# femto-dev/femto

Hardware: AMD Instinct MI355X
Metric: patterns/sec (count+locate) on 1 GiB index (higher is better)
Workload: dtype int64

## Files before the change

femto_amd/__init__.py:

```python
import ctypes as C
import os

import numpy as np

from . import build as _build

__all__ = ["Index", "Extractor", "FemtoAmdError", "lib", "ALPHA_SIZE", "CHARACTER_OFFSET", "Info"]

ALPHA_SIZE = 261
CHARACTER_OFFSET = 5
ERR_NAMES = {0: "NOERR", 1: "MEM", 2: "IO", 3: "PARAM", 4: "FORMAT", 5: "BZ_DATA", 6: "INVALID",
             8: "MISSING", 10: "FULL", 11: "OVERWORKED", 12: "UNKNOWN"}
ERR_PARAM, ERR_INVALID, ERR_FULL, ERR_OVERWORKED = 3, 6, 10, 11
BUDGET_ALL = -2


class FemtoAmdError(RuntimeError):
    def __init__(self, code, msg):
        super().__init__(f"femto_amd error {code} ({ERR_NAMES.get(code, '?')}): {msg}")
        self.code = code


class Info(C.Structure):
    _fields_ = [("total_length", C.c_int64), ("number_of_blocks", C.c_int64), ("number_of_documents", C.c_int64),
# ... 48 lines not shown
            v = lib().femto_amd_regexp_nfa(h).contents
            n, t = v.num_nodes, v.num_transitions

            def arr(p, count, ct):
                return np.ctypeslib.as_array(C.cast(p, C.POINTER(ct)), shape=(count,)).copy() if count else np.zeros(0, dtype=ct)

            return cls(arr(v.trans_start, n + 1, C.c_int32), arr(v.trans_char, t, C.c_int32), arr(v.trans_dest, t, C.c_int32),
                       arr(v.is_start, n, C.c_uint8), arr(v.is_final, n, C.c_uint8),
                       (v.cost_bound, v.subst_cost, v.delete_cost, v.insert_cost))
        finally:
            lib().femto_amd_regexp_free(h)

    @classmethod
    def from_query(cls, query, icase=False, streamline=True):
        q = np.frombuffer(bytes(query) + b"\0", dtype=np.uint8)
        h = C.c_void_p()
        _check(lib().femto_amd_query_compile(_ptr(q), len(query), (1 if icase else 0) | (0 if streamline else 2), C.byref(h)))
        try:
            v = lib().femto_amd_regexp_nfa(h).contents
            n, t = v.num_nodes, v.num_transitions

            def arr(p, count, ct):
                return np.ctypeslib.as_array(C.cast(p, C.POINTER(ct)), shape=(count,)).copy() if count else np.zeros(0, dtype=ct)

            a = cls(arr(v.trans_start, n + 1, C.c_int32), arr(v.trans_char, t, C.c_int32), arr(v.trans_dest, t, C.c_int32),
                    arr(v.is_start, n, C.c_uint8), arr(v.is_final, n, C.c_uint8),
                    (v.cost_bound, v.subst_cost, v.delete_cost, v.insert_cost))
            sp, sn = C.c_void_p(), C.c_int64(0)
            lit = None
            if lib().femto_amd_regexp_literal(h, C.byref(sp), C.byref(sn)):
                lit = arr(sp, sn.value, C.c_uint16)
            return a, lit, lib().femto_amd_regexp_echo(h)
        finally:
            lib().femto_amd_regexp_free(h)

    def struct(self):
        return NfaStruct(self.num_nodes, len(self.trans_char), self.trans_start.ctypes.data, self.trans_char.ctypes.data,
                         self.trans_dest.ctypes.data, self.is_start.ctypes.data, self.is_final.ctypes.data, *self.settings)


class NfaBatch:

    def __init__(self, nfas):
        self.nfas = list(nfas)
        self.n = len(self.nfas)
        self.arr = (NfaStruct * max(1, self.n))(*[a.struct() for a in self.nfas])


_lib = None


def lib():
    global _lib
    if _lib is None:
        if not os.path.exists(_build.LIB):
            raise ImportError(f"{_build.LIB} is missing: run `python -c 'import __graft_entry__ as g; g.build()'` "
                              "(there is no CPU fallback)")
        import sys
        if "torch" not in sys.modules:
            try:
                import torch
            except ImportError:
                pass
        L = C.CDLL(_build.LIB)
        vp, i64, i32 = C.c_void_p, C.c_int64, C.c_int
        L.femto_amd_open.argtypes = [C.c_char_p, i32, C.POINTER(vp)]
        L.femto_amd_close.argtypes = [vp]
        L.femto_amd_close.restype = None
        L.femto_amd_last_error.restype = C.c_char_p
        L.femto_amd_info.argtypes = [vp, C.POINTER(Info)]
        L.femto_amd_count_flat.argtypes = [vp, i64, vp, vp, vp, vp, vp]
        L.femto_amd_count_bytes.argtypes = [vp, i64, vp, vp, vp, vp, vp]
        L.femto_amd_locate_flat.argtypes = [vp, i64, vp, vp, vp, i32, vp, vp, vp, i64, C.POINTER(i64)]
        L.femto_amd_locate_flat_alloc.argtypes = [vp, i64, vp, vp, vp, i32, vp, vp, C.POINTER(vp), C.POINTER(i64)]
        L.femto_amd_parallel_locate_range.argtypes = [vp, i64, i64, vp]
        L.femto_amd_parallel_count.argtypes = [vp, i32, vp, vp, vp, vp]
        L.femto_amd_parallel_locate.argtypes = [vp, i32, vp, vp, i32, vp, vp]
        L.femto_amd_resolve_location.argtypes = [vp, i64, C.POINTER(i64), C.POINTER(i64)]
        L.femto_amd_document_info.argtypes = [vp, i64, C.POINTER(C.c_char_p), C.POINTER(i64)]
        L.femto_amd_count_device.argtypes = [vp, i64, vp, vp, vp, vp, vp, vp]
        L.femto_amd_locate_plan_device.argtypes = [vp, i64, vp, vp, vp, i32, vp, vp, vp, vp, vp]
        L.femto_amd_locate_walk_device.argtypes = [vp, i64, vp, vp, i64, vp, vp]
        L.femto_amd_locate_device.argtypes = [vp, i64, vp, vp, vp, i32, vp, vp, vp, vp, vp, i64, vp, vp]
        L.femto_amd_pack_counts_device.argtypes = [vp, i64, vp, vp, vp, vp, i64, vp, vp]
        L.femto_amd_trace_lines.argtypes = [vp, i64, vp, vp, vp, i32, vp, vp, C.POINTER(i64)]
        L.femto_amd_open_multi.argtypes = [C.c_char_p, i32, vp, C.POINTER(vp)]
        L.femto_amd_open_multi_striped.argtypes = [C.c_char_p, i32, vp, C.POINTER(vp)]
        L.femto_amd_striped_serve.argtypes = [vp, C.c_char_p, i32]
        L.femto_amd_open_striped_client.argtypes = [C.c_char_p, C.c_char_p, i32, i32, C.POINTER(vp)]
        L.femto_amd_multi_child.argtypes = [vp, i32, C.POINTER(vp)]
        L.femto_amd_device_count.argtypes = [vp]
        L.femto_amd_comm_unique_id.argtypes = [vp]
        L.femto_amd_comm_init.argtypes = [vp, vp, i32, i32]
        L.femto_amd_comm_gather.argtypes = [vp, vp, vp, i64, i32, vp]
        L.femto_amd_comm_info.argtypes = [vp, C.POINTER(i32), C.POINTER(i32)]
        L.femto_amd_regexp_search.argtypes = [vp, vp, i64, i64, vp, vp, vp, C.POINTER(i64)]
        L.femto_amd_regexp_search_approx.argtypes = [vp, vp, i64, i32, i32, i32, i32, i64, vp, vp, vp, vp, C.POINTER(i64)]
        L.femto_amd_regexp_match.argtypes = [vp, i64, vp, i64]
        L.femto_amd_options_init.argtypes = [vp]
        L.femto_amd_options_init.restype = None
        L.femto_amd_open_opts.argtypes = [C.c_char_p, i32, vp, C.POINTER(vp)]
        L.femto_amd_host_pipeline_stats.argtypes = [vp, vp]
        L.femto_amd_key_format.argtypes = [vp, C.POINTER(i32), C.POINTER(i32), vp]
        L.femto_amd_pack_keys_device.argtypes = [vp, i64, vp, vp, vp, vp, vp, vp]
        L.femto_amd_locate_keys_device.argtypes = [vp, i64, vp, i32, vp, vp, vp, vp, vp, vp, i64, vp, vp]
        L.femto_amd_regexp_compile.argtypes = [vp, i64, i32, i32, i32, i32, C.POINTER(vp)]
        L.femto_amd_regexp_nfa.argtypes = [vp]
        L.femto_amd_regexp_nfa.restype = C.POINTER(NfaStruct)
        L.femto_amd_regexp_free.argtypes = [vp]
        L.femto_amd_regexp_free.restype = None
        L.femto_amd_nfa_search_batch.argtypes = [vp, i64, vp, i64, vp, vp, vp, vp, vp, vp, C.POINTER(i64)]
        L.femto_amd_nfa_stats.argtypes = [vp, vp]
        if hasattr(L, "femto_amd_lf_steps_device"):
            L.femto_amd_lf_steps_device.argtypes = [vp, i64, vp, vp, vp, vp]
        L.femto_amd_key_table_id.argtypes = [vp, C.POINTER(C.c_uint64)]
        L.femto_amd_set_option.argtypes = [vp, C.c_char_p, i32]
        L.femto_amd_block_requests.argtypes = [vp, i64, vp, vp, vp, vp, vp]
        L.femto_amd_kernel_time_ms.argtypes = [vp, C.c_char_p, C.POINTER(C.c_double), C.POINTER(i64)]
        L.femto_amd_kernel_time_reset.argtypes = [vp]
        L.femto_amd_kernel_time_reset.restype = None
        L.femto_amd_kernel_time_enable.argtypes = [vp, i32]
        L.femto_amd_kernel_time_enable.restype = None
        L.femto_amd_build_index.argtypes = [C.c_char_p, i32, vp, vp, vp, C.c_char_p, i32]
        L.femto_amd_build_index_from_sa.argtypes = [C.c_char_p, i32, vp, vp, vp, C.c_char_p, vp]
        L.femto_amd_forward_steps.argtypes = [vp, i64, vp, vp, vp, vp]
        L.femto_amd_resolve_batch.argtypes = [vp, i64, vp, vp, vp]
        L.femto_amd_resolve_device.argtypes = [vp, vp, i64, vp, vp, vp, vp, vp]
        L.femto_amd_query_compile.argtypes = [vp, i64, i32, C.POINTER(vp)]
        L.femto_amd_regexp_literal.argtypes = [vp, C.POINTER(vp), C.POINTER(i64)]
        L.femto_amd_regexp_echo.argtypes = [vp]
        L.femto_amd_regexp_echo.restype = C.c_char_p
        L.femto_amd_query_echo.argtypes = [vp, i64, i32, i32, vp, i64]
        L.femto_amd_set_rank_mode.argtypes = [vp, i32]
        L.femto_amd_get_rank_mode.argtypes = [vp]
        L.femto_amd_pack_info.argtypes = [vp, C.POINTER(i32), C.POINTER(i64), C.POINTER(C.c_double), C.POINTER(i32)]
        L.femto_amd_structures.argtypes = [vp, vp, i32]
        L.femto_amd_flatten_index.argtypes = [C.c_char_p, C.c_char_p]
        L.femto_amd_bseq_encode.argtypes = [vp, i64, i32, vp, i64, C.POINTER(i64)]
        L.femto_amd_open_split.argtypes = [C.c_char_p, i32, i32, i32, C.POINTER(vp)]
        L.femto_amd_split_export.argtypes = [vp, vp]
        L.femto_amd_split_attach.argtypes = [vp, i32, vp]
        L.femto_amd_split_attach_local.argtypes = [vp, vp]
        L.femto_amd_split_commit.argtypes = [vp]
        L.femto_amd_split_info.argtypes = [vp, C.POINTER(i32), C.POINTER(i32), C.POINTER(i64), C.POINTER(i64)]
        L.femto_amd_extractor_open.argtypes = [vp, i32, i32, C.POINTER(vp)]
        L.femto_amd_extractor_free.argtypes = [vp]
        L.femto_amd_extractor_free.restype = None
        L.femto_amd_extractor_info.argtypes = [vp, C.POINTER(i32), C.POINTER(i32), C.POINTER(i64), C.POINTER(C.c_double)]
        L.femto_amd_extractor_eof_rows.argtypes = [vp, vp, i64]
        L.femto_amd_extract_device.argtypes = [vp, i64, vp, vp, vp, vp, vp]
        L.femto_amd_context_device.argtypes = [vp, i64, vp, vp, vp, i32, i32, vp, vp, vp]
        L.femto_amd_extract.argtypes = [vp, i64, vp, vp, vp, vp]
        L.femto_amd_context.argtypes = [vp, i64, vp, vp, i32, i32, vp, vp]
        L.femto_amd_extract_document.argtypes = [vp, i64, C.POINTER(vp), C.POINTER(i64)]
        L.femto_amd_doclist_info.argtypes = [C.POINTER(i32), C.POINTER(i32)]
        L.femto_amd_doclist_device.argtypes = [vp, i64, vp, vp, i64, vp, vp, vp, vp, vp, vp, vp, vp, vp, vp]
        L.femto_amd_docset_device.argtypes = [vp, i64, vp, vp, vp, vp, vp, vp, vp, vp, vp, i64, vp, vp]
        L.femto_amd_doclist.argtypes = [vp, i64, vp, vp, vp, i32, vp, C.POINTER(vp), C.POINTER(vp), C.POINTER(i64)]
        L.femto_amd_docset.argtypes = [vp, i64, vp, vp, vp, vp, vp, vp, vp, vp, C.POINTER(vp), C.POINTER(i64)]
        L.femto_amd_docpos_info.argtypes = [C.POINTER(i32)]
        L.femto_amd_docpos_device.argtypes = [vp, i64, vp, vp, vp, vp, vp, vp, vp, vp, vp, vp, vp, vp, vp, i64, vp, vp]
        L.femto_amd_docpos_documents_device.argtypes = [vp, i64, vp, vp, vp, vp, i64, vp, vp]
        L.femto_amd_docpos.argtypes = [vp, i64, vp, vp, vp, vp, vp, vp, vp, vp, vp, vp, vp, C.POINTER(vp), C.POINTER(vp), C.POINTER(i64)]
        L.femto_amd_proximity.argtypes = [vp, i64, vp, vp, vp, vp, vp, vp, vp, vp, i32, vp, C.POINTER(vp), C.POINTER(vp), C.POINTER(i64)]
        L.femto_amd_bquery_compile.argtypes = [vp, i64, i32, C.POINTER(vp)]
        L.femto_amd_bquery_info.argtypes = [vp, C.POINTER(i32), C.POINTER(i32), C.POINTER(i32)]
# ... 303 lines not shown
    def _pairs_back(n, res_starts, pd, po, total):
        if not total.value:
            return res_starts, np.zeros(0, dtype=np.int64), np.zeros(0, dtype=np.int64)
        try:
            return (res_starts, np.ctypeslib.as_array(C.cast(pd, C.POINTER(C.c_int64)), shape=(total.value,)).copy(),
                    np.ctypeslib.as_array(C.cast(po, C.POINTER(C.c_int64)), shape=(total.value,)).copy())
        finally:
            _libc_free(pd)
            _libc_free(po)

    def docpos(self, a_lists, b_lists, ops, distances):
        n = len(ops)

        def pack(lists):
            arrs = [np.asarray(x, dtype=np.int64).reshape(-1, 2) for x in lists]
            ln = np.array([len(x) for x in arrs], dtype=np.int32)
            st = np.zeros(n, dtype=np.int64)
            if n:
                st[1:] = np.cumsum(ln[:-1], dtype=np.int64)
            flat = np.concatenate(arrs) if n and ln.sum() else np.zeros((1, 2), dtype=np.int64)
            return np.ascontiguousarray(flat[:, 0]), np.ascontiguousarray(flat[:, 1]), st, ln

        (ad, ao, sa, na), (bd, bo, sb, nb) = pack(a_lists), pack(b_lists)
        op = np.ascontiguousarray(ops, dtype=np.int32)
        di = np.ascontiguousarray(distances, dtype=np.int32)
        res_starts = np.zeros(n + 1, dtype=np.int64)
        pd, po, total = C.c_void_p(), C.c_void_p(), C.c_int64(0)
        _check(lib().femto_amd_docpos(self._h, n, _ptr(ad), _ptr(ao), _ptr(sa), _ptr(na), _ptr(bd), _ptr(bo), _ptr(sb), _ptr(nb), _ptr(op),
                                      _ptr(di), _ptr(res_starts), C.byref(pd), C.byref(po), C.byref(total)))
        return self._pairs_back(n, res_starts, pd, po, total)

    def proximity(self, left, right, ops, distances, max_occs):
        n = len(ops)
        lp, lf, ls = flatten(left)
        rp, rf, rs = flatten(right)
        op = np.ascontiguousarray(ops, dtype=np.int32)
        di = np.ascontiguousarray(distances, dtype=np.int32)
        res_starts = np.zeros(n + 1, dtype=np.int64)
        pd, po, total = C.c_void_p(), C.c_void_p(), C.c_int64(0)
        _check(lib().femto_amd_proximity(self._h, n, _ptr(lp), _ptr(lf), _ptr(ls), _ptr(rp), _ptr(rf), _ptr(rs), _ptr(op), _ptr(di),
                                         int(max_occs), _ptr(res_starts), C.byref(pd), C.byref(po), C.byref(total)))
        return self._pairs_back(n, res_starts, pd, po, total)

    def bquery_run_batch(self, queries, max_occs):
        n = len(queries)
        handles = (C.c_void_p * max(1, n))(*[q._h for q in queries])
        res_starts = np.zeros(n + 1, dtype=np.int64)
        res_type = np.zeros(max(1, n), dtype=np.int32)
        pd, po, total = C.c_void_p(), C.c_void_p(), C.c_int64(0)
        _check(lib().femto_amd_bquery_run_batch(self._h, n, C.cast(handles, C.c_void_p), int(max_occs), _ptr(res_starts), _ptr(res_type),
                                                C.byref(pd), C.byref(po), C.byref(total)))
        return (res_starts, res_type[:n]) + self._pairs_back(n, res_starts, pd, po, total)[1:]

    def docpos_device(self, npairs, d_a_doc, d_a_off, d_a_start, d_a_n, d_b_doc, d_b_off, d_b_start, d_b_n, d_op, d_distance, d_res_starts,
                      d_res_doc, d_res_off, res_capacity, d_res_total, stream=0):
        _check(lib().femto_amd_docpos_device(self._h, int(npairs), d_a_doc or None, d_a_off or None, d_a_start or None, d_a_n or None,
                                             d_b_doc or None, d_b_off or None, d_b_start or None, d_b_n or None, d_op or None,
                                             d_distance or None, d_res_starts or None, d_res_doc or None, d_res_off or None,
                                             int(res_capacity), d_res_total or None, stream or None))

    def docpos_documents_device(self, nlists, d_starts, d_pair_doc, d_doc_starts, d_docs, doc_capacity, d_total, stream=0):
        _check(lib().femto_amd_docpos_documents_device(self._h, int(nlists), d_starts or None, d_pair_doc or None, d_doc_starts or None,
                                                       d_docs or None, int(doc_capacity), d_total or None, stream or None))

    def count_device(self, npats, d_plen, d_pats, d_starts, d_first, d_last, stream=0):
        _check(lib().femto_amd_count_device(self._h, npats, d_plen, d_pats, d_starts, d_first, d_last or None,
                                            stream or None))

    def locate_plan_device(self, npats, d_plen, d_pats, d_starts, max_occs, d_first, d_last, d_noccs, d_out_starts,
                           stream=0):
        _check(lib().femto_amd_locate_plan_device(self._h, npats, d_plen, d_pats, d_starts, max_occs, d_first, d_last,
                                                  d_noccs, d_out_starts, stream or None))

    def pack_counts_device(self, npats, d_first, d_last, d_counts8, d_big, big_capacity, d_big_n, stream=0):
        _check(lib().femto_amd_pack_counts_device(self._h, npats, d_first, d_last, d_counts8, d_big or None, big_capacity, d_big_n,
                                                  stream or None))

    def locate_walk_device(self, npats, d_first, d_out_starts, total, d_offsets, stream=0):
        _check(lib().femto_amd_locate_walk_device(self._h, npats, d_first, d_out_starts, total, d_offsets,
                                                  stream or None))

    def locate_device(self, npats, d_plen, d_pats, d_starts, max_occs, d_first, d_last, d_noccs, d_out_starts, d_offsets,
                      capacity, d_total, stream=0):
        _check(lib().femto_amd_locate_device(self._h, npats, d_plen, d_pats, d_starts, max_occs, d_first, d_last, d_noccs,
                                             d_out_starts, d_offsets, capacity, d_total, stream or None))

    TRACE_REGIONS = ("pack_lines", "level_table", "suffix_array", "level1_lines", "level2_lines", "text", "isa", "rank_units", "char_rank_lines",
                     "context_table")

    def trace_lines(self, npats, d_plen, d_pats, d_starts, max_occs):
        cl = np.zeros(10, dtype=np.int64)
        ll = np.zeros(10, dtype=np.int64)
        rows = C.c_int64(0)
        _check(lib().femto_amd_trace_lines(self._h, npats, d_plen, d_pats, d_starts, max_occs, _ptr(cl), _ptr(ll), C.byref(rows)))
        return dict(zip(self.TRACE_REGIONS, cl.tolist())), dict(zip(self.TRACE_REGIONS, ll.tolist())), rows.value

    def trace_reads(self):
        cr = np.zeros(10, dtype=np.int64)
        lr = np.zeros(10, dtype=np.int64)
        _check(lib().femto_amd_trace_reads(self._h, _ptr(cr), _ptr(lr)))
        return dict(zip(self.TRACE_REGIONS, cr.tolist())), dict(zip(self.TRACE_REGIONS, lr.tolist()))

    @staticmethod
    def comm_unique_id():
        blob = C.create_string_buffer(128)
        _check(lib().femto_amd_comm_unique_id(blob))
        return blob.raw

    def comm_init(self, id128, nranks, rank):
        _check(lib().femto_amd_comm_init(self._h, C.create_string_buffer(bytes(id128), 128), int(nranks), int(rank)))

    def comm_info(self):
        n, r = C.c_int(0), C.c_int(0)
        _check(lib().femto_amd_comm_info(self._h, C.byref(n), C.byref(r)))
        return {"nranks": n.value, "rank": r.value}

    def comm_gather(self, d_send, d_recv, bytes_per_rank, root=0, stream=0):
        _check(lib().femto_amd_comm_gather(self._h, d_send, d_recv or None, int(bytes_per_rank), int(root), stream or None))

    def key_format(self):
        bits, syms = C.c_int32(), C.c_int32()
        table = np.zeros(261, dtype=np.uint8)
        _check(lib().femto_amd_key_format(self._h, C.byref(bits), C.byref(syms), _ptr(table)))
        return bits.value, syms.value, table

    def lf_steps_device(self, n, d_rows, d_next, d_off, stream=0):
        _check(lib().femto_amd_lf_steps_device(self._h, int(n), d_rows, d_next, d_off, stream or None))

    def key_table_id(self):
        v = C.c_uint64(0)
        _check(lib().femto_amd_key_table_id(self._h, C.byref(v)))
        return v.value

    def pack_keys_device(self, npats, d_plen, d_pats, d_starts, d_keys, d_bad, stream=0):
        _check(lib().femto_amd_pack_keys_device(self._h, int(npats), d_plen, d_pats, d_starts, d_keys, d_bad, stream or None))

    def locate_keys_device(self, npats, d_keys, max_occs, d_ranges32, d_first, d_last, d_noccs, d_out_starts, d_offsets, capacity, d_total,
                           stream=0):
        _check(lib().femto_amd_locate_keys_device(self._h, int(npats), d_keys, int(max_occs), d_ranges32 or None, d_first or None,
                                                  d_last or None, d_noccs or None, d_out_starts or None, d_offsets or None,
                                                  int(capacity), d_total or None, stream or None))

    def nfa_search_batch(self, nfas, max_results=1 << 20):
        if isinstance(nfas, NfaBatch):
            n, arr = nfas.n, nfas.arr
        else:
            nfas = list(nfas)
            n = len(nfas)
            arr = (NfaStruct * max(1, n))(*[a.struct() for a in nfas])
        start = np.zeros(n + 1, dtype=np.int64)
        status = np.zeros(max(1, n), dtype=np.int32)
        m = max(0, int(max_results))
        first, last = np.zeros(max(1, m), dtype=np.int64), np.zeros(max(1, m), dtype=np.int64)
        mlen, cost = np.zeros(max(1, m), dtype=np.int32), np.zeros(max(1, m), dtype=np.int32)
        tot = C.c_int64(0)
        self.last_total = 0
        try:
            _check(lib().femto_amd_nfa_search_batch(self._h, n, C.cast(arr, C.c_void_p), m, _ptr(start), _ptr(first), _ptr(last), _ptr(mlen),
                                                    _ptr(cost), _ptr(status), C.byref(tot)))
        finally:
            self.last_total = tot.value
        k = tot.value if m else 0
        return start, first[:k], last[:k], mlen[:k], cost[:k], status[:n]

    def regexp_search_batch(self, regexes, max_results=1 << 20, approx=None):
        return self.nfa_search_batch([Nfa.from_regex(r, approx) for r in regexes], max_results)

# ... 212 lines not shown
```

femto_amd/build.py:

```python
import os
import subprocess
from concurrent.futures import ThreadPoolExecutor

HERE = os.path.dirname(os.path.abspath(__file__))
CSRC = os.path.join(HERE, "csrc")
EXTRACT = os.path.join(HERE, "extract")
DOCLIST = os.path.join(HERE, "doclist")
DOCPOS = os.path.join(HERE, "docpos")
BQUERY = os.path.join(HERE, "bquery")
OBJ = os.path.join(HERE, "_obj")
LIB = os.environ.get("FEMTO_AMD_LIB") or os.path.join(HERE, "libfemto_amd.so")
SOURCES = ["femto_amd_api.hip", "api_host.hip", "api_open.hip", "api_multi.hip", "regexp_search.hip", "resolve.hip", "trace_kernels.hip", "host_index.cpp", "index_builder.cpp", "suffix_sort.hip",
           "query_sort.hip", "host_pack.cpp", "../extract/extract.hip", "../doclist/doclist.hip", "../docpos/docpos.hip", "../bquery/bquery.hip"]
PLAIN_CXX = {"host_pack.cpp"}
CXX_FLAGS = ["-O3", "-std=c++17", "-fPIC", "-pthread"]
FLAGS = ["--offload-arch=gfx950", "-O3", "-std=c++17", "-fPIC", "-pthread", "-Wno-unused-result", "-Wno-cuda-compat"]
FLAGS += os.environ.get("FEMTO_AMD_EXTRA_FLAGS", "").split()
if os.environ.get("FEMTO_AMD_OBJ"):
    OBJ = os.environ["FEMTO_AMD_OBJ"]


def _headers():
    hs = [os.path.join(d, f) for d in (CSRC, EXTRACT, DOCLIST, DOCPOS, BQUERY) for f in os.listdir(d) if f.endswith((".hpp", ".h"))]
    hs.append(os.path.join(os.path.dirname(HERE), "include", "femto_amd.h"))
    return hs


def _newest_header():
    return max(os.path.getmtime(h) for h in _headers())


def _obj(src):
    return os.path.join(OBJ, os.path.splitext(os.path.basename(src))[0] + ".o")


def _stale(src, hdr_time):
    o = _obj(src)
    if not os.path.exists(o):
        return True
    t = os.path.getmtime(o)
    return os.path.getmtime(os.path.join(CSRC, src)) > t or hdr_time > t


def needs_build():
    if not os.path.exists(LIB):
        return True
    t = os.path.getmtime(LIB)
    if _newest_header() > t:
        return True
    return any(os.path.getmtime(os.path.join(CSRC, f)) > t for f in SOURCES)


def build(force=False, verbose=False):
    if not force and not needs_build():
        return LIB
    os.makedirs(OBJ, exist_ok=True)
    hdr_time = _newest_header()
    todo = [s for s in SOURCES if force or _stale(s, hdr_time)]

    def compile_one(src):
        if src in PLAIN_CXX:
            cmd = ["hipcc"] + CXX_FLAGS + ["-x", "c++", "-c", os.path.join(CSRC, src), "-o", _obj(src)]
        else:
            cmd = ["hipcc"] + FLAGS + ["-x", "hip", "-c", os.path.join(CSRC, src), "-o", _obj(src)]
        if verbose:
            print(" ".join(cmd), flush=True)
        subprocess.run(cmd, check=True)

    with ThreadPoolExecutor(max_workers=min(8, max(1, len(todo)))) as ex:
        list(ex.map(compile_one, todo))
    cmd = ["hipcc", "--offload-arch=gfx950", "-fPIC", "-shared", "-pthread", "-o", LIB] + [_obj(s) for s in SOURCES]
    if verbose:
        print(" ".join(cmd), flush=True)
    subprocess.run(cmd, check=True)
    return LIB


TOOL_SRC = os.path.join(os.path.dirname(HERE), "tools", "femto_amd_multiquery.cpp")
TOOL = os.path.join(HERE, "femto_amd_multiquery")


SEARCH_SRC = os.path.join(os.path.dirname(HERE), "tools", "femto_amd_search.cpp")
SEARCH = os.path.join(HERE, "femto_amd_search")


def build_tools(force=False, verbose=False):
    for src, exe in ((TOOL_SRC, TOOL), (SEARCH_SRC, SEARCH)):
        if not force and os.path.exists(exe) and os.path.getmtime(exe) > max(os.path.getmtime(src), os.path.getmtime(LIB)):
            continue
        cmd = ["g++", "-std=c++17", "-O2", "-o", exe, src, "-L" + HERE, "-lfemto_amd", "-Wl,-rpath,$ORIGIN",
               "-Wl,-rpath-link," + HERE, "-Wl,--allow-shlib-undefined"]
        if verbose:
            print(" ".join(cmd))
        subprocess.run(cmd, check=True)
    return TOOL


if __name__ == "__main__":
    build(force=True, verbose=True)
    build_tools(force=True, verbose=True)
```

include/femto_amd.h:

```cpp
#ifndef FEMTO_AMD_H
#define FEMTO_AMD_H

#include <stdint.h>
#include <stddef.h>

#ifdef __cplusplus
extern "C" {
#endif

enum {
  FEMTO_AMD_OK = 0,
  FEMTO_AMD_ERR_MEM = 1,
  FEMTO_AMD_ERR_IO = 2,
  FEMTO_AMD_ERR_PARAM = 3,
  FEMTO_AMD_ERR_FORMAT = 4,
  FEMTO_AMD_ERR_BZ_DATA = 5,
  FEMTO_AMD_ERR_INVALID = 6,
  FEMTO_AMD_ERR_MISSING = 8,
  FEMTO_AMD_ERR_FULL = 10,
  FEMTO_AMD_ERR_OVERWORKED = 11,
  FEMTO_AMD_ERR_UNKNOWN = 12
};

#define FEMTO_AMD_ALPHA_SIZE 261
#define FEMTO_AMD_CHARACTER_OFFSET 5

typedef struct femto_amd_index femto_amd_index_t;

int femto_amd_open(const char* index_path, int device, femto_amd_index_t** out);
void femto_amd_close(femto_amd_index_t* ix);

const char* femto_amd_last_error(void);

typedef struct {
  int64_t total_length;
  int64_t number_of_blocks;
  int64_t number_of_documents;
  int32_t block_size, bucket_size, mark_period, chunk_size;
  int32_t text_size_bits;
  int64_t total_buckets;
  int64_t image_bytes;
  int64_t table_bytes;
} femto_amd_info_t;
int femto_amd_info(const femto_amd_index_t* ix, femto_amd_info_t* out);


int femto_amd_parallel_count(femto_amd_index_t* ix, int npats, const int* plen,
                             const uint16_t* const* pats, int64_t* first, int64_t* last);

int femto_amd_parallel_locate(femto_amd_index_t* ix, int npats, const int* plen,
                              const uint16_t* const* pats, int max_occs_each,
                              int* noccs, int64_t** offsets);

int femto_amd_parallel_locate_range(femto_amd_index_t* ix, int64_t first, int64_t last, int64_t* offsets);

int femto_amd_count_flat(femto_amd_index_t* ix, int64_t npats, const int32_t* plen,
                         const uint16_t* pats, const int64_t* starts, int64_t* first, int64_t* last);
int femto_amd_locate_flat(femto_amd_index_t* ix, int64_t npats, const int32_t* plen,
                          const uint16_t* pats, const int64_t* starts, int max_occs_each,
                          int32_t* noccs, int64_t* out_starts, int64_t* offsets,
                          int64_t offsets_capacity, int64_t* total_out);

int femto_amd_locate_flat_alloc(femto_amd_index_t* ix, int64_t npats, const int32_t* plen,
                                const uint16_t* pats, const int64_t* starts, int max_occs_each,
                                int32_t* noccs, int64_t* out_starts, int64_t** offsets_out, int64_t* total_out);

int femto_amd_count_bytes(femto_amd_index_t* ix, int64_t npats, const int32_t* plen,
                          const uint8_t* bytes, const int64_t* starts, int64_t* first, int64_t* last);

int femto_amd_resolve_location(const femto_amd_index_t* ix, int64_t offset, int64_t* doc, int64_t* doc_offset);
int femto_amd_document_info(const femto_amd_index_t* ix, int64_t doc, const char** info, int64_t* len);

int femto_amd_resolve_batch(femto_amd_index_t* ix, int64_t n, const int64_t* offsets, int64_t* doc, int64_t* doc_offset);

int femto_amd_count_device(femto_amd_index_t* ix, int64_t npats, const int32_t* d_plen,
                           const uint16_t* d_pats, const int64_t* d_starts,
                           int64_t* d_first, int64_t* d_last, void* stream);

int femto_amd_locate_plan_device(femto_amd_index_t* ix, int64_t npats, const int32_t* d_plen,
                                 const uint16_t* d_pats, const int64_t* d_starts, int max_occs_each,
                                 int64_t* d_first, int64_t* d_last, int32_t* d_noccs,
                                 int64_t* d_out_starts, void* stream);
int femto_amd_locate_walk_device(femto_amd_index_t* ix, int64_t npats, const int64_t* d_first,
                                 const int64_t* d_out_starts, int64_t total, int64_t* d_offsets,
                                 void* stream);

int femto_amd_locate_device(femto_amd_index_t* ix, int64_t npats, const int32_t* d_plen,
                            const uint16_t* d_pats, const int64_t* d_starts, int max_occs_each,
                            int64_t* d_first, int64_t* d_last, int32_t* d_noccs, int64_t* d_out_starts,
                            int64_t* d_offsets, int64_t offsets_capacity, int64_t* d_total, void* stream);

int femto_amd_lf_steps_device(femto_amd_index_t* ix, int64_t n, const int64_t* d_rows, int64_t* d_next, int64_t* d_off, void* stream);

int femto_amd_resolve_device(femto_amd_index_t* ix, const int64_t* d_offsets, int64_t n, const int64_t* d_n, int64_t* d_doc,
                             int32_t* d_doc32, int64_t* d_doc_offset, void* stream);

typedef struct femto_amd_extractor femto_amd_extractor_t;
#define FEMTO_AMD_EXTRACT_FORCE_SAMPLES 1
#define FEMTO_AMD_EXTRACT_PATH_TEXT 0
#define FEMTO_AMD_EXTRACT_PATH_SAMPLES 1
int femto_amd_extractor_open(femto_amd_index_t* ix, int sample_shift , int flags, femto_amd_extractor_t** out);
void femto_amd_extractor_free(femto_amd_extractor_t* ex);
int femto_amd_extractor_info(const femto_amd_extractor_t* ex, int* path, int* sample_shift, int64_t* bytes, double* build_ms);
int femto_amd_extractor_eof_rows(const femto_amd_extractor_t* ex, int64_t* rows, int64_t n);
int femto_amd_extract_device(femto_amd_extractor_t* ex, int64_t n, const int64_t* d_pos, const int32_t* d_len,
                             const int64_t* d_out_starts, uint16_t* d_out, void* stream);
int femto_amd_context_device(femto_amd_extractor_t* ex, int64_t n, const int64_t* d_rows, const int64_t* d_offsets,
                             const int64_t* d_n, int before, int after, uint16_t* d_ctx, int64_t* d_pos_out, void* stream);
int femto_amd_extract(femto_amd_extractor_t* ex, int64_t n, const int64_t* pos, const int32_t* len, const int64_t* out_starts,
                      uint16_t* out);
int femto_amd_context(femto_amd_extractor_t* ex, int64_t n, const int64_t* rows, const int64_t* offsets, int before, int after,
                      uint16_t* ctx, int64_t* pos_out);
int femto_amd_extract_document(femto_amd_extractor_t* ex, int64_t doc, uint16_t** content, int64_t* len);

#define FEMTO_AMD_DOCSET_AND 0
#define FEMTO_AMD_DOCSET_OR 1
#define FEMTO_AMD_DOCSET_NOT 2
int femto_amd_doclist_info(int* wave_max, int* workgroup_max);
int femto_amd_doclist_device(femto_amd_index_t* ix, int64_t npats, const int64_t* d_out_starts, const int64_t* d_offsets,
                             int64_t capacity, const int64_t* d_total, int32_t* d_ndocs, int64_t* d_docs, int32_t* d_docs32,
                             int32_t* d_hits, int64_t* d_pair_doc, int64_t* d_pair_off, int64_t* d_doc_total, int32_t* d_status,
                             void* stream);
int femto_amd_docset_device(femto_amd_index_t* ix, int64_t npairs, const int64_t* d_docs_a, const int64_t* d_a_start,
                            const int32_t* d_a_n, const int64_t* d_docs_b, const int64_t* d_b_start, const int32_t* d_b_n,
                            const int32_t* d_op, int64_t* d_res_starts , int64_t* d_res_docs, int64_t res_capacity,
                            int64_t* d_res_total , void* stream);
int femto_amd_doclist(femto_amd_index_t* ix, int64_t npats, const int32_t* plen, const uint16_t* pats, const int64_t* starts,
                      int max_occs_each, int64_t* doc_starts , int64_t** docs, int32_t** hits, int64_t* total);
int femto_amd_docset(femto_amd_index_t* ix, int64_t npairs, const int64_t* docs_a, const int64_t* a_start, const int32_t* a_n,
                     const int64_t* docs_b, const int64_t* b_start, const int32_t* b_n, const int32_t* op,
                     int64_t* res_starts , int64_t** res_docs, int64_t* total);

#define FEMTO_AMD_DOCPOS_THEN 0
#define FEMTO_AMD_DOCPOS_WITHIN 1
#define FEMTO_AMD_DOCPOS_OR 2
int femto_amd_docpos_info(int* tile);
int femto_amd_docpos_device(femto_amd_index_t* ix, int64_t npairs, const int64_t* d_a_doc, const int64_t* d_a_off,
                            const int64_t* d_a_start, const int32_t* d_a_n, const int64_t* d_b_doc, const int64_t* d_b_off,
                            const int64_t* d_b_start, const int32_t* d_b_n, const int32_t* d_op, const int32_t* d_distance,
                            int64_t* d_res_starts , int64_t* d_res_doc, int64_t* d_res_off, int64_t res_capacity,
                            int64_t* d_res_total , void* stream);
int femto_amd_docpos_documents_device(femto_amd_index_t* ix, int64_t nlists, const int64_t* d_starts ,
                                      const int64_t* d_pair_doc, int64_t* d_doc_starts , int64_t* d_docs,
                                      int64_t doc_capacity, int64_t* d_total , void* stream);
int femto_amd_docpos(femto_amd_index_t* ix, int64_t npairs, const int64_t* a_doc, const int64_t* a_off, const int64_t* a_start,
                     const int32_t* a_n, const int64_t* b_doc, const int64_t* b_off, const int64_t* b_start, const int32_t* b_n,
                     const int32_t* op, const int32_t* distance, int64_t* res_starts , int64_t** res_doc,
                     int64_t** res_off, int64_t* total);
int femto_amd_proximity(femto_amd_index_t* ix, int64_t npairs, const int32_t* l_plen, const uint16_t* l_pats, const int64_t* l_starts,
                        const int32_t* r_plen, const uint16_t* r_pats, const int64_t* r_starts, const int32_t* op,
                        const int32_t* distance, int max_occs_each, int64_t* res_starts , int64_t** res_doc,
                        int64_t** res_off, int64_t* total);

int femto_amd_block_requests(femto_amd_index_t* ix, int64_t n, const int64_t* rows, const uint16_t* ch_in,
                             uint16_t* ch_out, int32_t* occ_out, int64_t* off_out);

int femto_amd_forward_steps(femto_amd_index_t* ix, int64_t n, const int64_t* rows, uint16_t* ch_out,
                            int64_t* row_out, int64_t* off_out);

int femto_amd_open_split(const char* index_path, int device, int part, int nparts, femto_amd_index_t** out);
int femto_amd_split_export(femto_amd_index_t* ix, void* blob128);
int femto_amd_split_attach(femto_amd_index_t* ix, int part, const void* blob128);
int femto_amd_split_attach_local(femto_amd_index_t* ix, femto_amd_index_t* owner);
int femto_amd_split_commit(femto_amd_index_t* ix);
int femto_amd_split_info(const femto_amd_index_t* ix, int* part, int* nparts, int64_t* seg_bytes, int64_t* image_bytes);

typedef struct femto_amd_nfa {
  int32_t num_nodes;
  int32_t num_transitions;
  const int32_t* trans_start;
  const int32_t* trans_char;
  const int32_t* trans_dest;
  const uint8_t* is_start;
// ... 141 lines not shown
```

Measured before the change: 19.31 billion.

## Add streamed persistent plan kernel fusing prefix-scan and SA locate walk

Adds a new locate path whose single persistent-wave kernel computes the exclusive prefix of per-pattern occurrence counts tile by tile and immediately expands each tile's occurrences into suffix-array lookups. It uses wave-level LDS binary search in place of the separate plan-rows scan and walk launches. Large-count patterns are handled by a follow-up big-rows kernel. The Python locate_device wrapper now calls the v2 entry point, so it runs by default. This is meant to cut kernel launches and intermediate global traffic, at the cost of serial per-wave tile processing and extra code complexity.

```diff
diff --git a/femto_amd/__init__.py b/femto_amd/__init__.py
--- a/femto_amd/__init__.py
+++ b/femto_amd/__init__.py
@@ -154,6 +154,7 @@
         L.femto_amd_locate_plan_device.argtypes = [vp, i64, vp, vp, vp, i32, vp, vp, vp, vp, vp]
         L.femto_amd_locate_walk_device.argtypes = [vp, i64, vp, vp, i64, vp, vp]
         L.femto_amd_locate_device.argtypes = [vp, i64, vp, vp, vp, i32, vp, vp, vp, vp, vp, i64, vp, vp]
+        L.femto_amd_locate_device_v2.argtypes = [vp, i64, vp, vp, vp, i32, vp, vp, vp, vp, vp, i64, vp, vp]
         L.femto_amd_pack_counts_device.argtypes = [vp, i64, vp, vp, vp, vp, i64, vp, vp]
         L.femto_amd_trace_lines.argtypes = [vp, i64, vp, vp, vp, i32, vp, vp, C.POINTER(i64)]
         L.femto_amd_open_multi.argtypes = [C.c_char_p, i32, vp, C.POINTER(vp)]
@@ -623,7 +624,7 @@
 
     def locate_device(self, npats, d_plen, d_pats, d_starts, max_occs, d_first, d_last, d_noccs, d_out_starts, d_offsets,
                       capacity, d_total, stream=0):
-        _check(lib().femto_amd_locate_device(self._h, npats, d_plen, d_pats, d_starts, max_occs, d_first, d_last, d_noccs,
+        _check(lib().femto_amd_locate_device_v2(self._h, npats, d_plen, d_pats, d_starts, max_occs, d_first, d_last, d_noccs,
                                              d_out_starts, d_offsets, capacity, d_total, stream or None))
 
     TRACE_REGIONS = ("pack_lines", "level_table", "suffix_array", "level1_lines", "level2_lines", "text", "isa", "rank_units", "char_rank_lines",
diff --git a/femto_amd/build.py b/femto_amd/build.py
--- a/femto_amd/build.py
+++ b/femto_amd/build.py
@@ -8,10 +8,11 @@
 DOCLIST = os.path.join(HERE, "doclist")
 DOCPOS = os.path.join(HERE, "docpos")
 BQUERY = os.path.join(HERE, "bquery")
+PLAN = os.path.join(HERE, "plan")
 OBJ = os.path.join(HERE, "_obj")
 LIB = os.environ.get("FEMTO_AMD_LIB") or os.path.join(HERE, "libfemto_amd.so")
 SOURCES = ["femto_amd_api.hip", "api_host.hip", "api_open.hip", "api_multi.hip", "regexp_search.hip", "resolve.hip", "trace_kernels.hip", "host_index.cpp", "index_builder.cpp", "suffix_sort.hip",
-           "query_sort.hip", "host_pack.cpp", "../extract/extract.hip", "../doclist/doclist.hip", "../docpos/docpos.hip", "../bquery/bquery.hip"]
+           "query_sort.hip", "host_pack.cpp", "../extract/extract.hip", "../doclist/doclist.hip", "../docpos/docpos.hip", "../bquery/bquery.hip", "../plan/plan_stream.hip"]
 PLAIN_CXX = {"host_pack.cpp"}
 CXX_FLAGS = ["-O3", "-std=c++17", "-fPIC", "-pthread"]
 FLAGS = ["--offload-arch=gfx950", "-O3", "-std=c++17", "-fPIC", "-pthread", "-Wno-unused-result", "-Wno-cuda-compat"]
@@ -21,7 +22,7 @@
 
 
 def _headers():
-    hs = [os.path.join(d, f) for d in (CSRC, EXTRACT, DOCLIST, DOCPOS, BQUERY) for f in os.listdir(d) if f.endswith((".hpp", ".h"))]
+    hs = [os.path.join(d, f) for d in (CSRC, EXTRACT, DOCLIST, DOCPOS, BQUERY, PLAN) for f in os.listdir(d) if f.endswith((".hpp", ".h"))]
     hs.append(os.path.join(os.path.dirname(HERE), "include", "femto_amd.h"))
     return hs
 
diff --git a/femto_amd/plan/plan_span.hpp b/femto_amd/plan/plan_span.hpp
--- /dev/null
+++ b/femto_amd/plan/plan_span.hpp
@@ -0,0 +1,45 @@
+#pragma once
+#include <cstdint>
+
+#if defined(__HIPCC__) || defined(__CUDACC__)
+#define PLAN_SPAN_FN __host__ __device__ inline
+#else
+#define PLAN_SPAN_FN inline
+#endif
+
+namespace femto_amd {
+
+constexpr int kPlanTile = 256;
+constexpr int kPlanWavesPerGroup = 4;
+constexpr int kPlanGroupsPerCu = 8;
+
+struct PlanSpan {
+  int64_t t0, t1;
+};
+
+PLAN_SPAN_FN int64_t plan_tiles(int64_t npats) { return npats <= 0 ? 0 : (npats + kPlanTile - 1) / kPlanTile; }
+
+PLAN_SPAN_FN PlanSpan plan_span_of(int64_t ntiles, int64_t nwaves, int64_t wave) {
+  if (ntiles <= 0 || nwaves <= 0 || wave < 0 || wave >= nwaves) return PlanSpan{0, 0};
+  const int64_t per = (ntiles + nwaves - 1) / nwaves;
+  const int64_t t0 = wave * per;
+  if (t0 >= ntiles) return PlanSpan{ntiles, ntiles};
+  const int64_t t1 = t0 + per < ntiles ? t0 + per : ntiles;
+  return PlanSpan{t0, t1};
+}
+
+PLAN_SPAN_FN int64_t plan_last_owner(int64_t ntiles, int64_t nwaves) {
+  if (ntiles <= 0 || nwaves <= 0) return -1;
+  const int64_t per = (ntiles + nwaves - 1) / nwaves;
+  return (ntiles - 1) / per;
+}
+
+PLAN_SPAN_FN int64_t plan_stream_groups(int64_t ntiles, int64_t num_cus, int64_t forced) {
+  if (ntiles <= 0) return 0;
+  int64_t g = forced > 0 ? forced : (num_cus > 0 ? num_cus : 1) * kPlanGroupsPerCu;
+  if (g > ntiles) g = ntiles;
+  if (g > 0x7fffffffLL) g = 0x7fffffffLL;
+  return g;
+}
+
+}
diff --git a/femto_amd/plan/plan_stream.hip b/femto_amd/plan/plan_stream.hip
--- /dev/null
+++ b/femto_amd/plan/plan_stream.hip
@@ -0,0 +1,301 @@
+#include <algorithm>
+#include <atomic>
+#include <cstdlib>
+
+#include "../csrc/api_internal.hpp"
+#include "../csrc/kernels.hip.hpp"
+#include "../csrc/pack_kernels.hip.hpp"
+#include "../csrc/ru_kernels.hip.hpp"
+#include "../csrc/pack2_kernels.hip.hpp"
+#include "../csrc/ind_kernels.hip.hpp"
+#include "../csrc/text_kernels.hip.hpp"
+#include "../csrc/ctx_kernels.hip.hpp"
+#include "../csrc/direct_kernels.hip.hpp"
+#include "plan_span.hpp"
+
+namespace femto_amd {
+namespace {
+
+struct alignas(16) I64x2 { int64_t x, y; };
+
+__device__ __forceinline__ void wave_lds_sync() {
+  __builtin_amdgcn_fence(__ATOMIC_RELEASE, "wavefront");
+  __builtin_amdgcn_wave_barrier();
+  __builtin_amdgcn_fence(__ATOMIC_ACQUIRE, "wavefront");
+}
+
+__device__ __forceinline__ int4 load_counts(const int32_t* __restrict__ noccs, int64_t npats, int64_t t, int64_t t1, int lane) {
+  int4 v = make_int4(0, 0, 0, 0);
+  if (t >= t1) return v;
+  const int64_t q0 = t * kPlanTile + 4 * lane;
+  if (q0 + 4 <= npats) {
+    v = *reinterpret_cast<const int4*>(noccs + q0);
+  } else {
+    if (q0 < npats) v.x = noccs[q0];
+    if (q0 + 1 < npats) v.y = noccs[q0 + 1];
+    if (q0 + 2 < npats) v.z = noccs[q0 + 2];
+  }
+  return v;
+}
+
+__device__ __forceinline__ void load_quad(const int64_t* __restrict__ a, bool vec, int64_t q0, const bool need[4], int64_t out[4]) {
+  if (vec) {
+    const I64x2 lo = *reinterpret_cast<const I64x2*>(a + q0), hi = *reinterpret_cast<const I64x2*>(a + q0 + 2);
+    out[0] = lo.x; out[1] = lo.y; out[2] = hi.x; out[3] = hi.y;
+  } else {
+#pragma unroll
+    for (int j = 0; j < 4; j++) out[j] = need[j] ? a[q0 + j] : 0;
+  }
+}
+
+template <bool kLong>
+__global__ __launch_bounds__(256) __attribute__((amdgpu_waves_per_eu(kLong ? 6 : 8, 8))) void plan_stream_kernel(
+    const int64_t npats, const int32_t* __restrict__ noccs, const int64_t* __restrict__ first, const PlanSums ps,
+    int64_t* __restrict__ out_starts, int64_t* __restrict__ offsets, const int64_t capacity, int* __restrict__ big_flag,
+    const DevIndex ix, int64_t* __restrict__ total_out, int64_t* __restrict__ total_user, const int64_t* __restrict__ sa_known) {
+  __shared__ uint32_t s_incl[kPlanWavesPerGroup][kPlanTile];
+  __shared__ int64_t s_first[kPlanWavesPerGroup][kPlanTile];
+  __shared__ int64_t s_lrel[kLong ? kPlanWavesPerGroup : 1][kLong ? kPlanTile : 1];
+  const int lane = threadIdx.x & 63, wv = threadIdx.x >> 6;
+  const int64_t nwaves = int64_t(gridDim.x) * kPlanWavesPerGroup, wave = int64_t(blockIdx.x) * kPlanWavesPerGroup + wv;
+  for (int64_t k = wave * 64 + lane; k < ps.next_words; k += nwaves * 64) ps.next_super[k] = 0;
+  const PlanSpan span = plan_span_of(ps.nblocks, nwaves, wave);
+  if (span.t0 >= span.t1) return;
+  int4 cur = load_counts(noccs, npats, span.t0, span.t1, lane);
+  int4 nx1 = load_counts(noccs, npats, span.t0 + 1, span.t1, lane);
+  int64_t base;
+  {
+    const int64_t b = span.t0, g = b >> 6;
+    uint64_t acc = lane < int(b & 63) ? uint64_t(ps.sums[(b & ~int64_t(63)) + lane]) : 0;
+    if (lane < int(g & 63)) acc += uint64_t(ps.super[(g & ~int64_t(63)) + lane]);
+    for (int64_t k = lane; k < (g >> 6); k += 64) acc += uint64_t(ps.super2[k]);
+    const uint64_t part = wave_sum_u64(acc);
+    const uint32_t lo = uint32_t(__shfl(int(uint32_t(part)), 0, 64)), hi = uint32_t(__shfl(int(uint32_t(part >> 32)), 0, 64));
+    base = int64_t((uint64_t(hi) << 32) | lo);
+  }
+  const bool first_vec = (reinterpret_cast<uintptr_t>(first) & 15u) == 0, known_vec = (reinterpret_cast<uintptr_t>(sa_known) & 15u) == 0;
+  for (int64_t t = span.t0; t < span.t1; t++) {
+    const int4 nx2 = load_counts(noccs, npats, t + 2, span.t1, lane);
+    const int64_t q0 = t * kPlanTile + 4 * lane;
+    const int64_t n[4] = {int64_t(cur.x), int64_t(cur.y), int64_t(cur.z), int64_t(cur.w)};
+    const int64_t lsum = n[0] + n[1] + n[2] + n[3];
+    int64_t incl = lsum;
+    if (kLong) {
+      uint64_t v = uint64_t(lsum);
+#pragma unroll
+      for (int d = 1; d < 64; d <<= 1) {
+        const uint32_t lo = uint32_t(__shfl_up(int(uint32_t(v)), d, 64)), hi = uint32_t(__shfl_up(int(uint32_t(v >> 32)), d, 64));
+        if (lane >= d) v += (uint64_t(hi) << 32) | lo;
+      }
+      incl = int64_t(v);
+    } else {
+      uint32_t v = uint32_t(lsum);
+#pragma unroll
+      for (int d = 1; d < 64; d <<= 1) {
+        const uint32_t y = uint32_t(__shfl_up(int(v), d, 64));
+        if (lane >= d) v += y;
+      }
+      incl = int64_t(v);
+    }
+    int64_t tile_rows;
+    if (kLong) {
+      const uint32_t lo = uint32_t(__shfl(int(uint32_t(uint64_t(incl))), 63, 64)), hi = uint32_t(__shfl(int(uint32_t(uint64_t(incl) >> 32)), 63, 64));
+      tile_rows = int64_t((uint64_t(hi) << 32) | lo);
+    } else {
+      tile_rows = int64_t(uint32_t(__shfl(int(uint32_t(incl)), 63, 64)));
+    }
+    const int64_t rel0 = incl - lsum;
+    const int64_t s0 = base + rel0, s1 = s0 + n[0], s2 = s1 + n[1], s3 = s2 + n[2];
+    if (q0 + 4 <= npats) {
+      *reinterpret_cast<I64x2*>(out_starts + q0) = I64x2{s0, s1};
+      *reinterpret_cast<I64x2*>(out_starts + q0 + 2) = I64x2{s2, s3};
+    } else {
+      if (q0 < npats) out_starts[q0] = s0;
+      if (q0 + 1 < npats) out_starts[q0 + 1] = s1;
+      if (q0 + 2 < npats) out_starts[q0 + 2] = s2;
+    }
+    if (offsets && tile_rows > 0) {
+      bool live[4], big[4];
+      bool any_big = false;
+#pragma unroll
+      for (int j = 0; j < 4; j++) {
+        big[j] = kLong && n[j] > kExpandSerialMax;
+        any_big |= big[j];
+        live[j] = q0 + j < npats && !big[j] && n[j] > 0;
+      }
+      if (kLong && any_big) atomicOr(big_flag, 1);
+      uint32_t mine[4], linc[4], lsum2 = 0;
+#pragma unroll
+      for (int j = 0; j < 4; j++) {
+        mine[j] = live[j] ? uint32_t(n[j]) : 0u;
+        lsum2 += mine[j];
+        linc[j] = lsum2;
+      }
+      uint32_t before = uint32_t(rel0);
+      if (kLong) {
+        uint32_t v = lsum2;
+#pragma unroll
+        for (int d = 1; d < 64; d <<= 1) {
+          const uint32_t y = uint32_t(__shfl_up(int(v), d, 64));
+          if (lane >= d) v += y;
+        }
+        before = v - lsum2;
+      }
+      *reinterpret_cast<uint4*>(&s_incl[wv][4 * lane]) = make_uint4(before + linc[0], before + linc[1], before + linc[2], before + linc[3]);
+      const uint32_t total = uint32_t(__shfl(int(before + lsum2), 63, 64));
+      bool need_known[4], need_first[4], want_known = false, want_first = false;
+      int64_t known[4] = {-1, -1, -1, -1}, f[4];
+#pragma unroll
+      for (int j = 0; j < 4; j++) {
+        need_known[j] = sa_known && mine[j] == 1u;
+        want_known |= need_known[j];
+      }
+      const bool whole = q0 + 4 <= npats;
+      if (want_known) load_quad(sa_known, whole && known_vec, q0, need_known, known);
+#pragma unroll
+      for (int j = 0; j < 4; j++) {
+        need_first[j] = mine[j] && !(need_known[j] && known[j] >= 0);
+        want_first |= need_first[j];
+      }
+      if (want_first) load_quad(first, whole && first_vec, q0, need_first, f);
+#pragma unroll
+      for (int j = 0; j < 4; j++) {
+        if (!need_first[j]) f[j] = (need_known[j] && known[j] >= 0) ? ~known[j] : 0;
+      }
+      *reinterpret_cast<I64x2*>(&s_first[wv][4 * lane]) = I64x2{f[0], f[1]};
+      *reinterpret_cast<I64x2*>(&s_first[wv][4 * lane + 2]) = I64x2{f[2], f[3]};
+      if (kLong) {
+        *reinterpret_cast<I64x2*>(&s_lrel[wv][4 * lane]) = I64x2{rel0, rel0 + n[0]};
+        *reinterpret_cast<I64x2*>(&s_lrel[wv][4 * lane + 2]) = I64x2{rel0 + n[0] + n[1], rel0 + n[0] + n[1] + n[2]};
+      }
+      wave_lds_sync();
+      for (uint32_t r0 = 0; r0 < total; r0 += 64) {
+        const uint32_t sidx = r0 + uint32_t(lane);
+        if (sidx < total) {
+          int lo = 0, hi = kPlanTile - 1;
+          while (lo < hi) {
+            const int mid = (lo + hi) >> 1;
+            if (s_incl[wv][mid] > sidx) hi = mid; else lo = mid + 1;
+          }
+          const uint32_t bef = lo ? s_incl[wv][lo - 1] : 0u;
+          const int64_t k = int64_t(sidx - bef);
+          const int64_t slot = base + (kLong ? s_lrel[wv][lo] : int64_t(bef)) + k;
+          if (slot < capacity) {
+            const int64_t fr = s_first[wv][lo], row = fr + k;
+            if (fr < 0) {
+              offsets[slot] = ~fr;
+            } else {
+              offsets[slot] = sa_at(ix, row);
+              trace_touch(ix, kTraceSa, sa_line_of(ix, row));
+            }
+          }
+        }
+      }
+      wave_lds_sync();
+    }
+    base += tile_rows;
+    cur = nx1;
+    nx1 = nx2;
+  }
+  if (span.t1 == ps.nblocks && lane == 0) {
+    total_out[0] = base;
+    total_out[1] = base > capacity ? 1 : 0;
+    if (total_user) {
+      total_user[0] = base;
+      total_user[1] = base > capacity ? 1 : 0;
+    }
+    out_starts[npats] = base;
+  }
+}
+
+std::atomic<int64_t> g_streamed{0}, g_fell_back{0}, g_big_launches{0}, g_last_groups{0};
+
+int launch_plan_stream(femto_amd_index* ix, Scratch& S, int64_t npats, const int32_t* d_noccs, const int64_t* d_first, int64_t* d_out_starts,
+                       int64_t* d_offsets, int64_t capacity, hipStream_t stream, const int64_t* d_sa_known, int max_occs, int64_t forced_groups) {
+  int* big_flag = S.d_flags + 1;
+  const int64_t ntiles = plan_tiles(npats);
+  const PlanSums ps = plan_sums_at(S.bsums.p, ntiles, false, S.bsums_parity);
+  S.bsums_clean = true;
+  const dim3 grid{uint32_t(plan_stream_groups(ntiles, ix->num_cus, forced_groups))}, block{uint32_t(kBlockThreads)};
+  const bool may_be_long = int64_t(max_occs) > kExpandSerialMax;
+  hipEvent_t e0 = nullptr, e1 = nullptr;
+  timer_begin(ix, ix->t_locate, stream, &e0, &e1);
+  if (may_be_long) {
+    hipLaunchKernelGGL(plan_stream_kernel<true>, grid, block, 0, stream, npats, d_noccs, d_first, ps, d_out_starts, d_offsets, capacity,
+                       big_flag, ix->dev, S.d_total, S.total_user, d_sa_known);
+    const dim3 bgrid{uint32_t(std::min<int64_t>(ntiles, int64_t(ix->num_cus) * 8))};
+    hipLaunchKernelGGL((plan_big_rows_kernel<kRowsSa, PackPolicy>), bgrid, block, 0, stream, npats, d_first, static_cast<const int2*>(nullptr),
+                       static_cast<const int64_t*>(d_out_starts), static_cast<const int64_t*>(S.d_total), capacity, d_offsets,
+                       static_cast<const int*>(big_flag), ix->dev);
+    g_big_launches++;
+  } else {
+    hipLaunchKernelGGL(plan_stream_kernel<false>, grid, block, 0, stream, npats, d_noccs, d_first, ps, d_out_starts, d_offsets, capacity,
+                       big_flag, ix->dev, S.d_total, S.total_user, d_sa_known);
+  }
+  HIP_TRY(hipGetLastError());
+  timer_end(ix, ix->t_locate, stream, e0, e1);
+  g_streamed++;
+  g_last_groups = int64_t(grid.x);
+  return 0;
+}
+
+}
+}
+
+int femto_amd_locate_device_v2(femto_amd_index_t* ix, int64_t npats, const int32_t* d_plen, const uint16_t* d_pats,
+                               const int64_t* d_starts, int max_occs_each, int64_t* d_first, int64_t* d_last,
+                               int32_t* d_noccs, int64_t* d_out_starts, int64_t* d_offsets, int64_t offsets_capacity,
+                               int64_t* d_total, void* stream_) {
+  API_BEGIN
+  if (!ix) return set_err(FEMTO_AMD_ERR_PARAM, "null index");
+  if (reinterpret_cast<uintptr_t>(d_pats) & 1u) return set_err(FEMTO_AMD_ERR_PARAM, "d_pats must be 2-byte aligned (uint16 symbols; the kernels read them in aligned 16-byte pieces)");
+  if (max_occs_each < 0 || offsets_capacity < 0) return set_err(FEMTO_AMD_ERR_PARAM, "negative max_occs_each / capacity");
+  const bool row_free = !d_first && !d_last;
+  if (npats && ((!row_free && (!d_first || !d_last)) || !d_noccs || !d_out_starts || !d_total)) return set_err(FEMTO_AMD_ERR_PARAM, "null argument");
+  int rc = ensure_device(ix);
+  if (rc) return rc;
+  hipStream_t stream = static_cast<hipStream_t>(stream_);
+  Lease L(ix, stream);
+  if (!L.s) return L.rc;
+  Scratch& S = *L.s;
+  Plan plan{max_occs_each, d_noccs, d_out_starts, offsets_capacity, false, d_total};
+  if (row_free && npats) {
+    if ((rc = S.first.reserve(size_t(npats + 1) * 8))) return rc;
+    d_first = S.first.as<int64_t>();
+    if (use_direct(ix)) {
+      plan.row_free = true;
+    } else {
+      if ((rc = S.last.reserve(size_t(npats + 1) * 8))) return rc;
+      d_last = S.last.as<int64_t>();
+    }
+  }
+  if ((rc = launch_count_plan(ix, S, npats, d_plen, d_pats, d_starts, d_first, d_last, &plan, stream))) return rc;
+  if (plan.done) {
+    const bool aligned = ((reinterpret_cast<uintptr_t>(d_noccs) | reinterpret_cast<uintptr_t>(d_out_starts)) & 15u) == 0;
+    const bool streamed = d_offsets && ix->dev.sa_full && aligned && npats > 0 && knob(-1, "FEMTO_AMD_PLAN_STREAM", 1) != 0;
+    if (streamed) {
+      const int64_t forced = knob(-1, "FEMTO_AMD_PLAN_STREAM_GRID", 0);
+      if ((rc = launch_plan_stream(ix, S, npats, d_noccs, d_first, d_out_starts, d_offsets, offsets_capacity, stream, plan.sa_known, max_occs_each, forced))) return rc;
+    } else {
+      if ((rc = launch_plan_rows(ix, S, npats, d_noccs, d_first, d_out_starts, d_offsets, offsets_capacity, stream, nullptr, true, plan.sa_known))) return rc;
+      g_fell_back++;
+    }
+  } else {
+    int64_t tot[2] = {0, 0};
+    HIP_TRY(hipMemcpyAsync(tot, S.d_total, sizeof tot, hipMemcpyDeviceToHost, stream));
+    HIP_TRY(hipStreamSynchronize(stream));
+    const int64_t walk = std::min(tot[0], offsets_capacity);
+    if (walk == tot[0] && d_offsets && (rc = launch_locate(ix, S, npats, d_first, d_out_starts, walk, d_offsets, stream))) return rc;
+    HIP_TRY(hipMemcpyAsync(d_total, S.d_total, 2 * sizeof(int64_t), hipMemcpyDeviceToDevice, stream));
+    g_fell_back++;
+  }
+  return FEMTO_AMD_OK;
+  API_END
+}
+
+void femto_amd_plan_stream_stats(int64_t out[4]) {
+  out[0] = g_streamed.load();
+  out[1] = g_fell_back.load();
+  out[2] = g_big_launches.load();
+  out[3] = g_last_groups.load();
+}
diff --git a/include/femto_amd.h b/include/femto_amd.h
--- a/include/femto_amd.h
+++ b/include/femto_amd.h
@@ -89,6 +89,11 @@
                             const uint16_t* d_pats, const int64_t* d_starts, int max_occs_each,
                             int64_t* d_first, int64_t* d_last, int32_t* d_noccs, int64_t* d_out_starts,
                             int64_t* d_offsets, int64_t offsets_capacity, int64_t* d_total, void* stream);
+int femto_amd_locate_device_v2(femto_amd_index_t* ix, int64_t npats, const int32_t* d_plen,
+                               const uint16_t* d_pats, const int64_t* d_starts, int max_occs_each,
+                               int64_t* d_first, int64_t* d_last, int32_t* d_noccs, int64_t* d_out_starts,
+                               int64_t* d_offsets, int64_t offsets_capacity, int64_t* d_total, void* stream);
+void femto_amd_plan_stream_stats(int64_t out[4]);
 
 int femto_amd_lf_steps_device(femto_amd_index_t* ix, int64_t n, const int64_t* d_rows, int64_t* d_next, int64_t* d_off, void* stream);
 
```

Result: faster. 20.60 billion, median of 6 (+6.7%).
